# GadGadGad/Convolutional-KAN-for-Image-Classification

Measured on AMD Instinct MI355X. Metric: images/sec fwd+bwd KAN-VGG11 3x32x32 bs=256/GPU, higher is better.
Workload: dtype f32

## Files before the change

### convolutional-kan-for-image-classification_amd/_lib.py

```python
from __future__ import annotations

import ctypes as C
import os
from typing import Optional

_HERE = os.path.dirname(os.path.abspath(__file__))
LIB_PATH = os.environ.get("KANCONV_LIB") or os.path.join(_HERE, "libkanconv.so")

KAN_MAX_PLANES = 16
KAN_MAX_TABLE = 32
KAN_FP_WORDS = 192
BASIS_BSPLINE, BASIS_RBF, BASIS_CHEBY, BASIS_POLY, BASIS_FOURIER, BASIS_RELU, BASIS_GRAM = 0, 1, 2, 3, 4, 5, 6
ACT_NONE, ACT_IDENTITY, ACT_GELU, ACT_SILU, ACT_RELU, ACT_TANH, ACT_SIGMOID, ACT_GELU_TANH = -1, 0, 1, 2, 3, 4, 5, 6


class KanGeom(C.Structure):
    _fields_ = [(n, C.c_int) for n in ("B", "C", "H", "W", "O", "Ho", "Wo", "kh", "kw", "sh", "sw", "ph", "pw", "dh", "dw", "groups")] + \
               [("x_bstride", C.c_longlong), ("y_bstride", C.c_longlong)]


class KanBasis(C.Structure):
    _fields_ = [("kind", C.c_int), ("n_basis", C.c_int), ("order", C.c_int), ("act", C.c_int),
                ("p0", C.c_float), ("p1", C.c_float), ("table", C.c_float * KAN_MAX_TABLE), ("chan_table", C.c_void_p)]


class KanPlan(C.Structure):
    _fields_ = [(n, C.c_int) for n in ("P", "K", "IPC", "KC", "Kpad", "Opad", "fwd_splits", "bwd_data_splits", "bwd_weight_splits",
                                          "fwd_target", "bwd_data_target", "bwd_weight_target", "x_pm_wanted", "dz_pm_wanted", "bwd_weight_expanded", "row_blocks", "e_pm_wanted", "fwd_expanded", "fwd_halo", "bwd_weight_halo",
                                          "fwd_band", "bwd_weight_band")] + \
               [(n, C.c_longlong) for n in ("packed_weight_bytes", "bwd_data_weight_bytes", "fwd_slab_elems", "bwd_data_slab_elems",
                                            "bwd_weight_slab_elems", "e_pm_elems")]


class KanWavGeom(C.Structure):
    _fields_ = [(n, C.c_int) for n in ("B", "C", "H", "W", "O", "Ho", "Wo", "kh", "kw", "sh", "sw", "ph", "pw", "dh", "dw", "wavelet")] + \
               [("x_bstride", C.c_longlong), ("u_bstride", C.c_longlong)]


WAVELETS = {"mexican_hat": 0, "morlet": 1, "dog": 2, "meyer": 3, "shannon": 4}

_P, _I, _LL, _F, _D = C.c_void_p, C.c_int, C.c_longlong, C.c_float, C.c_double
_GP, _BP = C.POINTER(KanGeom), C.POINTER(KanBasis)
SIGNATURES = {
    "kan_version": (C.c_char_p, []),
    "kan_last_error": (C.c_char_p, []),
    "kan_plan": (_I, [_GP, _BP, C.POINTER(KanPlan)]),
    "kan_pack_weights": (_I, [_P, _P, _P, _P, _GP, _BP, _P]),
    "kan_pack_cacheable": (_I, [_GP, _BP]),
    "kan_pack_weights_cached": (_I, [_P, _P, _P, _P, _GP, _BP, _P, _I, _I, _I, _P]),
    "kan_conv_fwd": (_I, [_P, _P, _P, _P, _GP, _BP, _P, _P]),
    "kan_position_major": (_I, [_P, _P, _I, _I, _I, _LL, _P]),
    "kan_conv_bwd_data": (_I, [_P, _P, _P, _P, _P, _P, _GP, _BP, _P, _P]),
    "kan_conv_bwd_data_params": (_I, [_P, _P, _P, _P, _P, _P, _P, _GP, _BP, _P, _P]),
    "kan_conv_bwd_weight": (_I, [_P, _P, _P, _P, _GP, _BP, _P, _P, _P]),
    "kan_position_major_expanded": (_I, [_P, _P, _GP, _BP, _P]),
    "kan_conv_fwd_expanded": (_I, [_P, _P, _P, _GP, _BP, _P]),
    "kan_conv_bwd_weight_expanded": (_I, [_P, _P, _P, _GP, _BP, _P]),
    "kan_unpack_wgrad": (_I, [_P, _P, _P, _GP, _BP, _P]),
    "kan_slab_reduce": (_I, [_P, _I, _LL, _P, _I, _I, _I, _LL, _P]),
    "kan_instnorm_prelu_fwd": (_I, [_P, _I, _LL, _P, _P, _P, _P, _P, _P, _P, _I, _I, _I, _LL, _F, _I, _P]),
    "kan_instnorm_prelu_bwd": (_I, [_P, _P, _P, _P, _P, _P, _P, _P, _P, _P, _P, _I, _I, _I, _LL, _I, _P]),
    "kan_instnorm_prelu_pool_fwd": (_I, [_P, _I, _LL, _P, _P, _P, _P, _P, _P, _P, _P, _I, _I, _I, _I, _LL, _F, _I, _P]),
    "kan_instnorm_prelu_pool_bwd": (_I, [_P, _P, _P, _P, _P, _P, _P, _P, _P, _P, _P, _P, _I, _I, _I, _I, _LL, _I, _P]),
    "kan_instnorm_prelu_poolk_fwd": (_I, [_P, _I, _LL, _P, _P, _P, _P, _P, _P, _P, _P, _I, _I, _I, _I, _LL, _F, _I, _I, _I, _P]),
    "kan_instnorm_prelu_poolk_bwd": (_I, [_P, _P, _P, _P, _P, _P, _P, _P, _P, _P, _P, _P, _I, _I, _I, _I, _LL, _I, _I, _I, _P]),
    "kan_split_supported": (_I, [C.POINTER(KanGeom), C.POINTER(KanBasis)]),
    "kan_split_weight_bytes": (_LL, [C.POINTER(KanGeom), C.POINTER(KanBasis)]),
    "kan_split_pack_weights": (_I, [_P, _P, _P, C.POINTER(KanGeom), C.POINTER(KanBasis), _P]),
    "kan_conv_fwd_split": (_I, [_P, _P, _P, C.POINTER(KanGeom), C.POINTER(KanBasis), _P]),
    "kan_wav_fwd": (_I, [_P, _P, _P, _P, _P, C.POINTER(KanWavGeom), _P]),
    "kan_wav_bwd_input": (_I, [_P, _P, _P, _P, _P, _P, C.POINTER(KanWavGeom), _P]),
    "kan_wav_param_workspace": (_LL, [C.POINTER(KanWavGeom)]),
    "kan_wav_bwd_params": (_I, [_P, _P, _P, _P, _P, _P, _P, _P, _P, C.POINTER(KanWavGeom), _P]),
    "kan_adamw_step": (_I, [_P, _P, _P, _P, _LL, _D, _D, _D, _D, _D, _I, _F, _P]),
    "kan_adamw_step_segments": (_I, [_P, _P, _P, _P, _P, _P, _P, _P, _P, _I, _I, _D, _D, _D, _D, _D, _I, _F, _P]),
}

_lib: Optional[C.CDLL] = None


class KanConvError(RuntimeError):
# ... 27 lines not shown
```

### convolutional-kan-for-image-classification_amd/csrc/kan_internal.h

```cpp
#pragma once
#include <type_traits>
#include "kanconv.h"

int kan_fail_msg(const char* fmt, const char* a);
int kan_raise_lds_limit(const void* kernel, int bytes);

enum : int {
    FAST_GENERIC = 0,
    FAST_BSPLINE_SILU = 1,
    FAST_BSPLINE_GELU = 2,
    FAST_RBF8 = 3,
    FAST_CHEBY5 = 4,
    FAST_CHEBY4 = 5,
    FAST_POLY4 = 6,
    FAST_POLY3 = 7,
    FAST_RBF5 = 8,
    FAST_RELU8 = 9,
    FAST_GRAM4 = 10,
    FAST_POLY1 = 11,
    FAST_LAST = 11
};
enum : unsigned {
    ON_TAP_MAJOR = 1u << 0,
    ON_BIG_TILES = 1u << 1,
    ON_HALO_FWD = 1u << 2,
    ON_HALO_BWD_WEIGHT = 1u << 3,
    ON_BAND_FWD = 1u << 4,
    ON_BAND_BWD_WEIGHT = 1u << 5,
    ON_EXPANDED_FWD = 1u << 6,
    ON_EXPANDED = 1u << 7,
    ON_ROWBLK_BWD_DATA = 1u << 8,
};
constexpr unsigned fast_routes(int f) {
    constexpr unsigned bspline = ON_TAP_MAJOR | ON_BIG_TILES | ON_HALO_FWD | ON_HALO_BWD_WEIGHT | ON_BAND_FWD | ON_BAND_BWD_WEIGHT |
                                 ON_EXPANDED_FWD | ON_EXPANDED | ON_ROWBLK_BWD_DATA;
    switch (f) {
        case FAST_BSPLINE_SILU: case FAST_BSPLINE_GELU: return bspline;
        case FAST_RBF8: return ON_TAP_MAJOR | ON_BAND_FWD | ON_BAND_BWD_WEIGHT;
        case FAST_CHEBY5: return ON_TAP_MAJOR | ON_BIG_TILES | ON_BAND_FWD | ON_BAND_BWD_WEIGHT;
        case FAST_CHEBY4: return ON_TAP_MAJOR | ON_HALO_FWD | ON_BAND_FWD;
        case FAST_POLY4: return ON_TAP_MAJOR | ON_BIG_TILES | ON_HALO_FWD | ON_BAND_FWD;
        case FAST_POLY3: case FAST_RBF5: case FAST_POLY1: return ON_TAP_MAJOR;
        case FAST_RELU8: return ON_HALO_FWD | ON_HALO_BWD_WEIGHT | ON_EXPANDED_FWD | ON_EXPANDED;
        case FAST_GRAM4: return ON_HALO_FWD | ON_HALO_BWD_WEIGHT | ON_EXPANDED;
        default: return 0;
    }
}
constexpr bool fast_has(int f, unsigned routes) { return (fast_routes(f) & routes) == routes && f != FAST_GENERIC; }
constexpr int fast_kind(int f) {
    return (f == FAST_RBF8 || f == FAST_RBF5) ? KAN_BASIS_RBF : (f == FAST_CHEBY5 || f == FAST_CHEBY4) ? KAN_BASIS_CHEBY
         : (f == FAST_POLY4 || f == FAST_POLY3 || f == FAST_POLY1) ? KAN_BASIS_POLY : f == FAST_RELU8 ? KAN_BASIS_RELU
         : f == FAST_GRAM4 ? KAN_BASIS_GRAM : KAN_BASIS_BSPLINE;
}
constexpr int fast_kc(int f) { return fast_kind(f) == KAN_BASIS_BSPLINE || fast_kind(f) == KAN_BASIS_RBF ? 18 : 16; }

template <int V> using IC = std::integral_constant<int, V>;
template <unsigned ROUTES, int F = 1, class Fn>
bool dispatch_fast(int f, Fn&& fn) {
    if constexpr (F > FAST_LAST) {
        return false;
    } else {
        if constexpr (fast_has(F, ROUTES)) {
            if (f == F) { fn(IC<F>{}); return true; }
        }
        return dispatch_fast<ROUTES, F + 1>(f, fn);
    }
}
template <int V, int... REST, class Fn>
// ... 23 lines not shown
    int lds_bytes, wgs_per_cu;
    int fwd_splits;
    int bw_ok, bw_WR, bw_NI, bw_NT, bw_tiles_o, bw_row_tiles, bw_TPI, bw_ptiles, bw_cells, bw_slots, bw_lds_bytes, bw_splits;
    unsigned short bw_ph_rt0[KAN_BAND_MAX_PHASES + 1];
    unsigned char ph_a[KAN_BAND_MAX_PHASES], ph_b[KAN_BAND_MAX_PHASES];
    short ph_tap0[KAN_BAND_MAX_PHASES + 1];
    unsigned short tap_shift[KAN_BAND_MAX_TAPS];
    unsigned short tap_rt[KAN_BAND_MAX_TAPS];
    short tap_step[KAN_BAND_MAX_TAPS], tap_nt[KAN_BAND_MAX_TAPS];
} KanBandCfg;

void kan_band_cfg(const KanGeom* g, const KanBasis* b, int fast, KanBandCfg* cfg);
int kan_band_bwd_weight_launch(const float* dz, const float* x, const float* xn, float* dwp, const KanGeom* g, const KanBasis* b,
                               const KanBandCfg* cfg, int splits, long long slab_elems, void* stream);
int kan_band_fwd_launch(const float* x, const float* xn, const float* wp, float* z, const KanGeom* g, const KanBasis* b,
                        const KanBandCfg* cfg, int splits, long long slab_elems, void* stream);

constexpr int DW_T = 9;
constexpr int DW_MAX_TP = 96;

enum class Route { TAP_MAJOR, DW, BAND, HALO, EXPANDED };

struct FwdCfg { int TO, TP, tiles_o, tiles_p, chunks, splits, slots; };
struct BdCfg { int CH, tiles_c, tiles_p, n_ob, Opad32, chunks, splits; };
struct BwCfg { int TR, TO, tiles_r, tiles_o, chunks, splits, slots; };
struct BwHaloCfg { int R, nimg, spb, n_bands, tiles_r, tiles_o, splits, bands_per_split; };

struct ConvPlan {
    KanPlan pub;
    int fast;
    Route fwd, bwd_data, bwd_weight;
    bool pm_fwd, pm_bwd_data, pm_bwd_weight;
    bool rowblk_bwd_data;
    bool pmdma_xcd, pm_lpt, pm_xcd;
    FwdCfg fc;
    BdCfg bd;
    BwCfg bw;
    BwHaloCfg bwh;
    KanBandCfg band;
};
int plan_conv(const KanGeom* g, const KanBasis* b, ConvPlan* cp);

int live_taps_out(const KanGeom* g, int hw);
int live_taps_in(const KanGeom* g, int hw);
int live_positions_for_tap(const KanGeom* g, int tap);
int balance_tiles(const int* weight, int n, unsigned short* idx);
```

### convolutional-kan-for-image-classification_amd/csrc/kan_plan.hip

```cpp
#include <hip/hip_runtime.h>
#include <cstdio>
#include <cstdlib>
#include <cstring>
#include "kanconv.h"
#include "kan_device.h"
#include "kan_common.h"
#include "kan_internal.h"

namespace {

int fail(const char* msg) { return kan_fail_msg("%s", msg); }

int check(const KanGeom* g, const KanBasis* b) {
    if (!g || !b) return fail("null geometry/basis");
    if (g->groups < 0 || g->groups > 65535) return fail("groups out of range");
    if (g->B <= 0 || g->C <= 0 || g->O <= 0 || g->H <= 0 || g->W <= 0 || g->Ho <= 0 || g->Wo <= 0) return fail("non-positive dimension");
    if (g->kh <= 0 || g->kw <= 0 || g->sh <= 0 || g->sw <= 0 || g->dh <= 0 || g->dw <= 0 || g->ph < 0 || g->pw < 0) return fail("bad conv parameters");
    if (g->kh > 255 || g->kw > 255 || g->C > 65535) return fail("kernel size / channel count out of supported range");
    if ((g->H + 2 * g->ph - g->dh * (g->kh - 1) - 1) / g->sh + 1 != g->Ho || (g->W + 2 * g->pw - g->dw * (g->kw - 1) - 1) / g->sw + 1 != g->Wo)
        return fail("Ho/Wo inconsistent with H/W, kernel, stride, padding, dilation");
    if ((long long)g->B * g->Ho * g->Wo >= (1ll << 31) || (long long)g->B * g->H * g->W >= (1ll << 31)) return fail("pixel count exceeds int32");
    if ((long long)g->B * g->x_bstride * 4 >= (1ll << 31) || (long long)g->B * g->y_bstride * 4 >= (1ll << 31))
        return fail("activation tensors must be smaller than 2 GiB (32-bit buffer offsets)");
    if (g->x_bstride < (long long)ngroups(g) * g->C * g->H * g->W || g->y_bstride < (long long)ngroups(g) * g->O * g->Ho * g->Wo)
// ... 94 lines not shown
    if (g->kh != 3 || g->kw != 3 || g->sh != 1 || g->sw != 1 || g->dh != 1 || g->dw != 1 || g->ph != 1 || g->pw != 1) return false;
    if ((g->C & 1) || g->O % 128 != 0) return false;
    if (pm_fwd) return false;
    const int W = g->W, H = g->H;
    return (W == 32 && H % 4 == 0) || (W == 16 && H % 8 == 0) || (W == 8 && H == 8) || (W == 4 && H == 4);
}
bool band_fwd(const KanGeom* g, const KanBasis* b, int f, bool dw, bool pm_fwd, bool halo, KanBandCfg* out) {
    if (tuning_off("KAN_BAND") || !fast_has(f, ON_BAND_FWD)) return false;
    if (b->kind == KAN_BASIS_POLY && b->order == 0) return false;
    if (dw || pm_fwd || halo) return false;
    if (!(g->C <= 3 || round_up(g->O, 64) % 128 != 0 || (g->kh * g->kw >= 4 && g->C % 2 == 0 && !tuning_off("KAN_BAND_WIDE")))) return false;
    kan_band_cfg(g, b, f, out);
    return out->ok != 0;
}
FwdCfg fwd_cfg(const KanGeom* g, const KanPlan& pl, bool big, bool pm_fwd, bool halo) {
    FwdCfg c;
    c.TO = (big && !pm_fwd) ? 256 : (pl.Opad % 128 == 0) ? 128 : 64;
    c.slots = c.TO == 256 ? 512 : 1024;
    c.TP = 128;
    c.tiles_o = pl.Opad / c.TO;
    c.tiles_p = ceil_div((long long)g->B * g->Ho * g->Wo, c.TP);
    c.chunks = pl.Kpad / pl.KC;
    c.splits = pick_splits((long long)c.tiles_o * c.tiles_p * ngroups(g), c.chunks, 8, 4.0 * g->B * g->O * g->Ho * g->Wo * ngroups(g), c.slots);
    if (halo) {
        const int n_pairs = g->C / 2, pps = ceil_div(n_pairs, c.splits < n_pairs ? c.splits : n_pairs);
        c.splits = ceil_div(n_pairs, pps);
    }
    return c;
}
bool rowblk_bwd_data(const KanGeom* g, int f, bool pm_bwd_data) {
    return !tuning_off("KAN_BD_ROWBLK") && fast_has(f, ON_ROWBLK_BWD_DATA) && !pm_bwd_data && g->H == 4 && g->W == 4 && g->Ho == 4 && g->Wo == 4 &&
           g->kh == 3 && g->kw == 3 && g->sh == 1 && g->sw == 1 && g->ph == 1 && g->pw == 1 && g->dh == 1 && g->dw == 1 && g->B % 8 == 0 && g->O % 16 == 0;
}
struct LiveClass { long long tiles; int live_steps; };

int pick_target_steps(const LiveClass* cls, int ncls, int min_steps, double slab_bytes, int* max_splits, long long SLOTS = 1024) {
    int hi = 1;
    for (int i = 0; i < ncls; ++i) if (cls[i].live_steps > hi) hi = cls[i].live_steps;
    int best = hi; double best_cost = -1; int best_ms = 1;
    for (int t = min_steps < hi ? min_steps : hi; t <= hi; ++t) {
        long long wgs = 0; int ms = 1;
        for (int i = 0; i < ncls; ++i) {
            const int sp = cls[i].live_steps > 0 ? ceil_div(cls[i].live_steps, t) : 1;
            wgs += cls[i].tiles * sp;
            if (sp > ms) ms = sp;
        }
        const long long rounds = (wgs + SLOTS - 1) / SLOTS;
        const double cost = (double)(rounds * (t + 6)) + ms * slab_cost_steps(slab_bytes);
        if (best_cost < 0 || cost < best_cost) { best_cost = cost; best = t; best_ms = ms; }
    }
    *max_splits = best_ms;
    return best;
}
BdCfg bd_cfg(const KanGeom* g, const KanPlan& pl) {
    BdCfg c;
    c.CH = 64 / pl.P;
    c.tiles_c = ceil_div(g->C, 2 * c.CH);
    c.tiles_p = ceil_div((long long)g->B * g->H * g->W, 128);
    c.n_ob = ceil_div(g->O, 16);
    c.Opad32 = round_up(g->O, 32);
    c.chunks = g->kh * g->kw * c.n_ob;
    c.splits = pick_splits((long long)c.tiles_c * c.tiles_p * ngroups(g), c.chunks, 8, 4.0 * g->B * g->C * g->H * g->W * ngroups(g));
    return c;
}
bool pmdma_bwd_weight(const KanGeom* g, const KanBasis* b, int f, bool want_pm_bw) {
    if (tuning_off("KAN_PMDMA") || !fast_has(f, ON_EXPANDED)) return false;
// ... 98 lines not shown
        order[j] = v;
    }
    for (int r = 0; r < n; ++r) {
        const int depth = r / 8, k = r % 8, bin = (depth & 1) ? 7 - k : k;
        int slot = depth * 8 + bin;
        if (slot >= n) slot = r;
        idx[slot] = (unsigned short)order[r];
    }
    bool seen[PERM_MAX] = {false};
    for (int i = 0; i < n; ++i) { if (idx[i] >= n || seen[idx[i]]) return 0; seen[idx[i]] = true; }
    return n;
}

int plan_conv(const KanGeom* g, const KanBasis* b, ConvPlan* cp) {
    if (int rc = check(g, b)) return rc;
    ConvPlan& c = *cp;
    KanPlan* pl = &c.pub;
    const int T = g->kh * g->kw, G = ngroups(g), f = fast_variant(b);
    c.fast = f;
    const bool pm_shape = pmdma_fwd_shape(g, f);
    c.pm_fwd = want_pix_major(g, b, PM_FWD, pm_shape);
    c.pm_bwd_data = want_pix_major(g, b, PM_BWD_DATA, false);
    const bool want_pm_bw = want_pix_major(g, b, PM_BWD_WEIGHT, false);
    const bool dw = dw_direct(g, b);
    const bool halo = halo_fwd(g, b, f, c.pm_fwd);
    c.band.ok = c.band.bw_ok = 0;
    const bool band = band_fwd(g, b, f, dw, c.pm_fwd, halo, &c.band);
    const bool pmdma_fwd = pm_shape && c.pm_fwd;
    const bool pmdma_bw = pmdma_bwd_weight(g, b, f, want_pm_bw);
    const bool halo_bw = halo_bwd_weight(g, f, pmdma_bw);
    c.pm_bwd_weight = want_pm_bw && !halo_bw;
    const bool band_bw = band && c.band.bw_ok && !want_pm_bw && !tuning_off("KAN_BAND_BW");
    c.rowblk_bwd_data = rowblk_bwd_data(g, f, c.pm_bwd_data);
    c.pmdma_xcd = tuning_on("KAN_PMDMA_XCD");
    c.pm_lpt = !tuning_off("KAN_PM_LPT");
    c.pm_xcd = !tuning_off("KAN_PM_XCD");
    c.fwd = dw ? Route::DW : band ? Route::BAND : halo ? Route::HALO : pmdma_fwd ? Route::EXPANDED : Route::TAP_MAJOR;
    c.bwd_data = dw ? Route::DW : Route::TAP_MAJOR;
    c.bwd_weight = dw ? Route::DW : band_bw ? Route::BAND : halo_bw ? Route::HALO : pmdma_bw ? Route::EXPANDED : Route::TAP_MAJOR;
    pl->P = b->n_basis + (b->act != KAN_ACT_NONE);
    pl->K = g->C * T * pl->P;
    {
        int i18 = 18 / pl->P, i16 = 16 / pl->P;
        if (i18 > 4) i18 = 4;
        if (i16 > 4) i16 = 4;
        const bool use18 = (long long)i18 * pl->P * 16 > (long long)i16 * pl->P * 18;
        pl->KC = use18 ? 18 : 16;
        pl->IPC = use18 ? i18 : i16;
        if (pl->P >= 10 && pl->P <= 12) { pl->KC = 12; pl->IPC = 1; }
        if (halo) { pl->KC = 2 * pl->P; pl->IPC = 2; }
    }
    pl->Kpad = ceil_div(g->C * T, pl->IPC) * pl->KC;
    if (band) { pl->KC = c.band.NPLE; pl->IPC = c.band.NG; pl->Kpad = c.band.n_steps * c.band.NPLE; }
    pl->Opad = round_up(g->O, 64);
    pl->packed_weight_bytes = (long long)G * pl->Kpad * pl->Opad * 4;
    c.bd = bd_cfg(g, *pl);
    pl->bwd_data_weight_bytes = (long long)G * T * c.bd.Opad32 * c.bd.tiles_c * 128 * 4;
    pl->fwd_slab_elems = (long long)g->B * g->y_bstride;
    pl->bwd_data_slab_elems = (long long)g->B * g->x_bstride;
    pl->bwd_weight_slab_elems = (long long)G * pl->K * pl->Opad;
    const bool big = big_tiles(f, *pl);
    c.fc = fwd_cfg(g, *pl, big, c.pm_fwd, halo);
    c.bw = bw_cfg(g, *pl, big, c.pm_bwd_weight);
    if (halo_bw) c.bwh = bw_halo_cfg(g, *pl);
    pl->fwd_splits = band ? c.band.fwd_splits : c.fc.splits;
    pl->bwd_data_splits = c.bd.splits;
// ... 45 lines not shown
```

### convolutional-kan-for-image-classification_amd/csrc/kanconv.hip

```cpp
#include <hip/hip_runtime.h>
#include <cstdio>
#include <cstdlib>
#include <cstring>
#include <cmath>
#include <cstdint>
#include <mutex>
#include <type_traits>
#include <vector>
#include "kanconv.h"
#include "kan_device.h"

#include "kan_common.h"
#include "kan_internal.h"

namespace {


thread_local char g_err[512] = "";
int fail(const char* fmt, const char* a = "") {
    snprintf(g_err, sizeof(g_err), fmt, a);
    return -1;
}
}
int kan_fail_msg(const char* fmt, const char* a) { return fail(fmt, a); }
// ... 557 lines not shown
            for (int r = 0; r < 16; ++r) {
                const int o = o_tile0 + w_o * 64 + mi * 32 + mfma_row(r, lane);
                if (o < g.O) zb[(size_t)o * HoWo] = acc[mi][ni][r];
            }
        }
    }
}

template <int M>
__device__ __forceinline__ void wave_reduce_scatter(float (&v)[M], int lane, int& idx, float& tot) {
    int base = 0;
    int m = M;
#pragma unroll
    for (int off = 32; off >= 1; off >>= 1) {
        if (m > 1) {
            const int h = m / 2;
            const bool up = (lane & off) != 0;
#pragma unroll
            for (int i = 0; i < M / 2; ++i) {
                if (i < h) {
                    const float keep = up ? v[h + i] : v[i], send = up ? v[i] : v[h + i];
                    v[i] = keep + __shfl_xor(send, off, 64);
                }
            }
            base += up ? h : 0;
            m = h;
        } else {
            v[0] += __shfl_xor(v[0], off, 64);
        }
    }
    idx = base; tot = v[0];
}

template <int KIND, int FAST, int RB = 0>
__global__ __launch_bounds__(256, 4) void k_conv_bwd_data(
    const float* __restrict__ dz, const float* __restrict__ x, const float* __restrict__ xn, const float* __restrict__ wd,
    float* __restrict__ dx, float* __restrict__ dxn, DevGeom g, DevBasis bs, int CH, int n_ct, int n_ob, int Opad16,
    int n_chunks, int chunks_per_split, long long slab_elems, unsigned dz_bytes, TilePerm perm, float* __restrict__ dpar) {
    constexpr int TP = 128, KD = 16, NT = 256;
    __shared__ __attribute__((aligned(16))) float smem[2 * 2 * KD * 128];
    __shared__ float sTab[KAN_MAX_TABLE];

    const int tid = threadIdx.x, lane = tid & 63;
    const int wave = __builtin_amdgcn_readfirstlane(tid >> 6);
    const int w_r = wave >> 1, w_p = wave & 1;
    const int HoWo = g.Ho * g.Wo, HW = g.H * g.W, P = bs.P;
    const int Min = g.B * HW;
    const BlockId blk = xcd_block_order(false);
    const int grp = blk.y / n_ct;
    const int px_tile0 = (perm.n ? (int)perm.idx[blk.x] : blk.x) * TP, ct = blk.y - grp * n_ct;
    const int ncol = n_ct * 128;
    const int pxl = (wave & 1) * 64 + lane, ol0 = wave >> 1;
    const bool idle_rows = (ct * 2 + w_r) * CH >= g.C;
    {
        const size_t xo = (size_t)grp * g.C * HW;
        x += xo; xn += xo; dx += xo; if (dxn) dxn += xo;
        dz += (size_t)grp * g.O * HoWo * (g.pix_major ? g.B : 1);
        wd += (size_t)grp * (g.kh * g.kw) * Opad16 * ncol;
    }

    if (tid < KAN_MAX_TABLE) sTab[tid] = bs.tab[tid];
    const int my_px = px_tile0 + (RB ? ((pxl >> 2) & 7) * 16 + (pxl >> 5) * 4 + (pxl & 3) : pxl);
    const bool pv = my_px < Min;
    int pb, ph_, pw_;
    {
        int hw;
        if (g.pix_major) { hw = my_px / g.B; pb = my_px - hw * g.B; }
        else { pb = my_px / HW; hw = my_px - pb * HW; }
        ph_ = hw / g.W; pw_ = hw - ph_ * g.W;
    }
    const kan_rsrc dz_rs = make_rsrc(dz, dz_bytes);
    const unsigned dz_img = g.pix_major ? (unsigned)pb : (unsigned)pb * (unsigned)g.ybs;
    const unsigned zstride = g.pix_major ? (unsigned)g.B : 1u;
    const int wv = wave;

    int cur_tap = -1; unsigned base = KAN_OOB;
    const unsigned wlane = (unsigned)((lane >> 5) * ncol + (lane & 31) * 4) * 4u;
    const unsigned row_bytes = (unsigned)HoWo * zstride * 4u;
    const bool o_full = (n_ob * KD == g.O);

    auto issue = [&](int ch, int buf) {
        const int tap = ch / n_ob, o0 = (ch - tap * n_ob) * KD;
        if (tap != cur_tap) {
            cur_tap = tap;
            const int r = tap / g.kw, t = tap - r * g.kw;
            const int hn = ph_ + g.ph - r * g.dh, wn = pw_ + g.pw - t * g.dw;
            int ho = hn, wo = wn; bool ok = pv && hn >= 0 && wn >= 0;
            if (g.sh != 1 || g.sw != 1) {
                ho = hn / g.sh; wo = wn / g.sw;
                ok = ok && ho * g.sh == hn && wo * g.sw == wn;
            }
            ok = ok && ho < g.Ho && wo < g.Wo;
            base = ok ? (dz_img + (unsigned)(ho * g.Wo + wo) * zstride) * 4u : KAN_OOB;
        }
        float* dW = smem + buf * (2 * KD * 128);
// ... 65 lines not shown
#pragma unroll
        for (int b = 0; b < 2; ++b)
#pragma unroll
            for (int r = 0; r < 16; ++r) acc[a][b][r] = 0.f;

    int ch0 = blk.z * chunks_per_split;
    int ch1 = min(n_chunks, ch0 + chunks_per_split);
    unsigned tapmask = 0xffffffffu;
    if (g.pix_major) {
        tapmask = 0;
        const int T = g.kh * g.kw;
        const int hwA = px_tile0 / g.B, hwB = min(px_tile0 + TP - 1, Min - 1) / g.B;
        for (int hw = hwA; hw <= hwB; ++hw)
            for (int tap = 0; tap < T; ++tap) tapmask |= (tap_alive_in(g, hw, tap) ? 1u : 0u) << tap;
        auto seg = [&](int tap) { return tap * n_ob; };
        const int L = live_step_count(tapmask, T, n_chunks, seg);
        const int S = min((int)gridDim.z, max(1, (L + chunks_per_split - 1) / chunks_per_split));
        if (blk.z >= S) { ch0 = ch1 = n_chunks; }
        else {
            ch0 = blk.z == 0 ? 0 : live_step_pos(tapmask, T, n_chunks, (int)((long long)L * blk.z / S), seg);
            ch1 = blk.z == S - 1 ? n_chunks : live_step_pos(tapmask, T, n_chunks, (int)((long long)L * (blk.z + 1) / S), seg);
        }
    }
    auto next_live = [&](int ch) -> int {
        if (!g.pix_major) return ch;
        while (ch < ch1) {
            const int tap = ch / n_ob;
            if ((tapmask >> tap) & 1u) return ch;
            ch = (tap + 1) * n_ob;
        }
        return ch1;
    };
    int ch = next_live(ch0);
    if (ch < ch1) { if (RB) issue_rb(ch, 0); else issue(ch, 0); }
    const int ar = w_r * 64 + (lane & 31), bp = w_p * 64 + (lane & 31), kh2 = lane >> 5;
    for (int cur = 0; ch < ch1; cur ^= 1) {
        asm volatile("s_waitcnt vmcnt(0)" ::: "memory");
        __syncthreads();
        const bool mixed_now = pend_mixed;
        ch = next_live(ch + 1);
        if (ch < ch1) { if (RB) issue_rb(ch, cur ^ 1); else issue(ch, cur ^ 1); }
        const float* cW = smem + cur * (2 * KD * 128);
        const float* cG = cW + KD * 128;
        const unsigned aw = lds_addr(cW + kh2 * 128 + ar), ag = lds_addr(cG + kh2 * TP + bp);
        if (RB) {
            const bool l0b = !(mixed_now && w_p == 0), l1a = !(mixed_now && w_p == 1);
            if (!idle_rows) KAN_MFMA_STEP_LIVE(KD / 2, aw, 128, ag, TP, true, l0b, l1a, true);
        } else if (!idle_rows) KAN_MFMA_STEP(KD / 2, aw, 128, ag, TP);
    }

    const bool same_in = (x == xn);
    const bool split_out = (dxn != nullptr);
    float* dxs = dx + (size_t)blk.z * slab_elems;
    float* dxns = split_out ? dxn + (size_t)blk.z * slab_elems : nullptr;
    if (FAST == 3 || FAST == 8) {
        constexpr int FP = FAST == 3 ? 9 : 6, FCH = 64 / FP, NIT = (FCH + 1) / 2;
        const float inv_d = 1.0f / bs.p0;
#pragma unroll 1
        for (int half = 0; half < 2; ++half) {
            float xv[NIT], nv[NIT]; unsigned ok = 0;
#pragma unroll
            for (int it = 0; it < NIT; ++it) {
                const int cl = ol0 + 2 * it, c = (ct * 2 + half) * FCH + cl;
                const bool v = cl < FCH && c < g.C && pv;
                const size_t idx = (size_t)pb * g.xbs + (size_t)c * HW + (size_t)(ph_ * g.W + pw_);
                xv[it] = v ? x[idx] : 0.f;
                nv[it] = v ? xn[idx] : 0.f;
                ok |= (v ? 1u : 0u) << it;
// ... 1676 lines not shown
    if (pl.KC != pl.IPC * pl.P || (pl.fwd_band && pack_needs_clear(g, pl))) {
        if (hipMemsetAsync(wp, 0, (size_t)pl.packed_weight_bytes, st) != hipSuccess) return fail("memset failed");
    } else if (!pl.fwd_band && NI % pl.IPC != 0) {
        if (G > 1) {
            if (hipMemsetAsync(wp, 0, (size_t)pl.packed_weight_bytes, st) != hipSuccess) return fail("memset failed");
        } else {
            size_t off = (size_t)(pl.Kpad - pl.KC) * pl.Opad;
            if (hipMemsetAsync(wp + off, 0, (size_t)pl.KC * pl.Opad * 4, st) != hipSuccess) return fail("memset failed");
        }
    }
    const int nb_base = hb ? ceil_div(g->C * T, 32) : 0;
    const int tiles_x = nb_base + ceil_div(g->C * b->n_basis * T, 32), tiles_y = pl.Opad / 32;
    const long long n_tiles = (long long)tiles_x * tiles_y;
    const long long cap = fp ? 1024 : 4096;
    dim3 grid((unsigned)(n_tiles < cap ? n_tiles : cap), 1, G);
    hipLaunchKernelGGL(k_pack, grid, dim3(256), 0, st, w_base, w_basis, wp, q, nb_base, wp_gs, tiles_x, tiles_y, fp, fp_cur);
    if (wd && cp.bwd_data == Route::DW) {
        if (hipMemcpyAsync(wd, wp, (size_t)pl.packed_weight_bytes, hipMemcpyDeviceToDevice, st) != hipSuccess) return fail("memcpy failed");
    } else if (wd) {
        const BdCfg& c = cp.bd;
        const int bx = c.tiles_c * 4, by = c.Opad32 / 32 * G;
        const long long nt = (long long)bx * by;
        const long long capd = fp ? 128 : 1024;
        dim3 gd((unsigned)(nt < capd ? nt : capd), 1, T);
        hipLaunchKernelGGL(k_pack_bwd_data, gd, dim3(256), 0, st, (const float*)wp, wd, q, c.CH, c.tiles_c, c.Opad32, wp_gs, bx, by, fp, fp_cur);
    }
    return launch_ok("pack");
}

int kan_pack_weights(const float* w_base, const float* w_basis, float* wp, float* wd, const KanGeom* g, const KanBasis* b, void* stream) {
    return pack_weights_impl(w_base, w_basis, wp, wd, g, b, nullptr, 0, stream);
}

int kan_pack_cacheable(const KanGeom* g, const KanBasis* b) {
    ConvPlan cp;
    if (plan_conv(g, b, &cp)) return 0;
    if ((long long)g->O * g->C * (b->n_basis + 1) * g->kh * g->kw >= (1ll << 31)) return 0;
    return (!pack_needs_clear(g, cp.pub) && cp.fwd != Route::DW && ngroups(g) == 1) ? 1 : 0;
}

int kan_pack_weights_cached(const float* w_base, const float* w_basis, float* wp, float* wd, const KanGeom* g, const KanBasis* b,
                            unsigned long long* ring, int cur, int force, int sample_stride, void* stream) {
    static_assert(KAN_FP_WORDS == 3 * FP_LANES, "ring size");
    if (!ring || cur < 0 || cur > 2 || sample_stride < 1) return fail("bad fingerprint ring arguments");
    if (!kan_pack_cacheable(g, b)) return fail("cached packing is not offered for this geometry (kan_pack_cacheable)");
    const int hb = b->act != KAN_ACT_NONE;
    if ((hb && !w_base) || !w_basis) return fail("null weight pointer");
    if (((size_t)w_basis & 15) || (hb && ((size_t)w_base & 15))) return fail("cached packing needs 16-byte aligned weight tensors");
    const int T = g->kh * g->kw;
    const long long na = hb ? (long long)g->O * g->C * T : 0, nbs = (long long)g->O * g->C * b->n_basis * T;
    const long long groups4 = ((na + 3) / 4 + (nbs + 3) / 4 + sample_stride - 1) / sample_stride;
    long long blocks = (groups4 + 256 * 8 - 1) / (256 * 8); if (blocks > 4096) blocks = 4096; if (blocks < 1) blocks = 1;
    hipLaunchKernelGGL(k_fingerprint, dim3((unsigned)blocks), dim3(256), 0, (hipStream_t)stream, hb ? w_base : w_basis, (unsigned)na, w_basis,
                       (unsigned)nbs, (unsigned)sample_stride, ring, cur);
    if (int rc = launch_ok("fingerprint")) return rc;
    return pack_weights_impl(w_base, w_basis, wp, wd, g, b, force ? nullptr : ring, cur, stream);
}

int kan_unpack_wgrad(const float* dwp, float* dw_base, float* dw_basis, const KanGeom* g, const KanBasis* b, void* stream) {
    ConvPlan cp;
    if (int rc = plan_conv(g, b, &cp)) return rc;
    const KanPlan& pl = cp.pub;
    const int hb = b->act != KAN_ACT_NONE;
    if ((hb && !dw_base) || !dw_basis || !dwp) return fail("null weight-gradient pointer");
    hipStream_t st = (hipStream_t)stream;
    const int T = g->kh * g->kw, G = ngroups(g);
// ... 121 lines not shown
    ConvPlan cp;
    if (int rc = plan_conv(g, b, &cp)) return rc;
    const KanPlan& pl = cp.pub;
    if (dpar && cp.bwd_data == Route::DW) return fail("kan_conv_bwd_data_params: depthwise layers take the weight-gradient route");
    if (!dz || !x || !xn || !wd || !dx) return fail("null tensor pointer");
    if ((b->kind == KAN_BASIS_RELU || b->kind == KAN_BASIS_GRAM) && !b->chan_table) return fail("ReLU / Gram bases need their device parameter table (chan_table)");
    if (!dxn && x != xn) return fail("dxn is required when xn != x");
    hipStream_t st = (hipStream_t)stream;
    if (cp.bwd_data == Route::DW) {
        DevGeom dgd = dev_geom(g); DevBasis dbd = dev_basis(b);
        dim3 grid(ceil_div((long long)g->B * g->H * g->W, 256), ngroups(g));
        dispatch_kind(b->kind, [&](auto kind) {
            hipLaunchKernelGGL((k_dw_bwd_data<decltype(kind)::value>), grid, dim3(256), 0, st, dz, x, xn, wd, dx, dxn, dgd, dbd, pl.Opad, pl.IPC, pl.KC, pl.Kpad);
        });
        return launch_ok("dw_bwd_data");
    }
    const BdCfg& c = cp.bd;
    DevGeom dg = dev_geom(g);
    dg.pix_major = (dz_pm && cp.pm_bwd_data) ? 1 : 0;
    if (dg.pix_major) dz = dz_pm;
    DevBasis db = dev_basis(b);
    if ((long long)c.tiles_c * ngroups(g) > 65535) return fail("groups * channel tiles exceed the grid limit");
    dim3 grid(c.tiles_p, c.tiles_c * ngroups(g), pl.bwd_data_splits);
    const int cps = dg.pix_major ? pl.bwd_data_target : ceil_div(c.chunks, pl.bwd_data_splits);
    TilePerm perm; perm.n = 0;
    if (dg.pix_major) perm = tile_perm(c.tiles_p, [&](int t) {
        const int hw = (int)(((long long)t * 128) / g->B);
        return ceil_div(live_taps_in(g, hw < g->H * g->W ? hw : 0) * c.n_ob, cps > 0 ? cps : 1);
    });
    const int fv = cp.fast;
    const int fast = (fv == FAST_RBF8 || fv == FAST_RBF5) ? ((x != xn && dxn) ? fv : 0) : ((x == xn && !dxn) ? fv : 0);
    const bool rb = !dg.pix_major && cp.rowblk_bwd_data;
    const unsigned dz_bytes = (unsigned)((long long)g->B * g->y_bstride * 4);
    auto launch = [&](auto kind, auto fast, auto rbv) {
        hipLaunchKernelGGL((k_conv_bwd_data<decltype(kind)::value, decltype(fast)::value, decltype(rbv)::value>), grid, dim3(256), 0, st, dz, x, xn, wd,
                           dx, dxn, dg, db, c.CH, c.tiles_c, c.n_ob, c.Opad32, c.chunks, cps, pl.bwd_data_slab_elems, dz_bytes, perm, dpar);
    };
    const bool launched = dispatch_fast<ON_TAP_MAJOR>(fast, [&](auto fv) {
        constexpr int F = decltype(fv)::value;
        if constexpr (fast_has(F, ON_ROWBLK_BWD_DATA)) {
            if (rb) return launch(IC<fast_kind(F)>{}, fv, IC<1>{});
        }
        launch(IC<fast_kind(F)>{}, fv, IC<0>{});
    });
    if (!launched) dispatch_kind(b->kind, [&](auto kind) { launch(kind, IC<FAST_GENERIC>{}, IC<0>{}); });
    return launch_ok("conv_bwd_data");
}

int kan_conv_bwd_weight(const float* dz, const float* x, const float* xn, float* dwp, const KanGeom* g, const KanBasis* b,
                        const float* x_pm, const float* dz_pm, void* stream) {
    ConvPlan cp;
    if (int rc = plan_conv(g, b, &cp)) return rc;
    const KanPlan& pl = cp.pub;
    if (!dz || !x || !xn || !dwp) return fail("null tensor pointer");
    if ((b->kind == KAN_BASIS_RELU || b->kind == KAN_BASIS_GRAM) && !b->chan_table) return fail("ReLU / Gram bases need their device parameter table (chan_table)");
    hipStream_t st = (hipStream_t)stream;
    if (cp.bwd_weight == Route::DW) {
        DevGeom dgd = dev_geom(g); DevBasis dbd = dev_basis(b);
        dim3 grid(pl.bwd_weight_splits, ngroups(g));
        dispatch_kind(b->kind, [&](auto kind) {
            hipLaunchKernelGGL((k_dw_bwd_weight<decltype(kind)::value>), grid, dim3(256), 0, st, dz, x, xn, dwp, dgd, dbd, pl.K, pl.Opad, pl.bwd_weight_slab_elems);
        });
        return launch_ok("dw_bwd_weight");
    }
    if (cp.bwd_weight == Route::BAND) {
        if (x != xn && b->kind != KAN_BASIS_RBF && b->kind != KAN_BASIS_POLY) return fail("this basis / activation pair runs on single-input kernels: pass xn == x");
        return kan_band_bwd_weight_launch(dz, x, xn, dwp, g, b, &cp.band, pl.bwd_weight_splits, pl.bwd_weight_slab_elems, stream);
    }
    const unsigned x_bytes = (unsigned)((long long)g->B * g->x_bstride * 4), dz_bytes = (unsigned)((long long)g->B * g->y_bstride * 4);
    if (cp.bwd_weight == Route::HALO) {
        if (x != xn) return fail("internal: the channel-major weight-gradient layout needs x == xn");
        const BwHaloCfg& hc = cp.bwh;
        const DevGeom dgh = dev_geom(g); const DevBasis dbh = dev_basis(b);
        if ((long long)hc.tiles_o * ngroups(g) > 65535) return fail("groups * output tiles exceed the grid limit");
        dim3 grid(hc.tiles_r, hc.tiles_o * ngroups(g), hc.splits);
        dispatch_fast<ON_HALO_BWD_WEIGHT>(cp.fast, [&](auto fv) {
            auto launch = [&](auto w, auto r, auto nimg) {
                hipLaunchKernelGGL((k_conv_bwd_weight_halo<decltype(fv)::value, decltype(w)::value, decltype(r)::value, decltype(nimg)::value>), grid,
// ... 286 lines not shown
```

### include/kanconv.h

```cpp
#ifndef KANCONV_H
#define KANCONV_H

#ifdef __cplusplus
extern "C" {
#endif

#define KAN_MAX_PLANES 16
#define KAN_MAX_TABLE  32
#define KAN_FP_WORDS   192

enum { KAN_BASIS_BSPLINE = 0, KAN_BASIS_RBF = 1, KAN_BASIS_CHEBY = 2, KAN_BASIS_POLY = 3, KAN_BASIS_FOURIER = 4, KAN_BASIS_RELU = 5, KAN_BASIS_GRAM = 6 };
enum { KAN_ACT_NONE = -1, KAN_ACT_IDENTITY = 0, KAN_ACT_GELU = 1, KAN_ACT_SILU = 2, KAN_ACT_RELU = 3,
       KAN_ACT_TANH = 4, KAN_ACT_SIGMOID = 5, KAN_ACT_GELU_TANH = 6 };

typedef struct KanGeom {
    int B, C, H, W;
    int O, Ho, Wo;
    int kh, kw, sh, sw, ph, pw, dh, dw;
    int groups;
    long long x_bstride;
    long long y_bstride;
} KanGeom;

typedef struct KanBasis {
// ... 5 lines not shown

typedef struct KanPlan {
    int P;
    int K;
    int IPC, KC;
    int Kpad, Opad;
    int fwd_splits;
    int bwd_data_splits;
    int bwd_weight_splits;
    int fwd_target, bwd_data_target, bwd_weight_target;
    int x_pm_wanted, dz_pm_wanted;
    int bwd_weight_expanded;
    int row_blocks;
    int e_pm_wanted, fwd_expanded;
    int fwd_halo, bwd_weight_halo;
    int fwd_band, bwd_weight_band;
    long long packed_weight_bytes;
    long long bwd_data_weight_bytes;
    long long fwd_slab_elems;
    long long bwd_data_slab_elems;
    long long bwd_weight_slab_elems;
    long long e_pm_elems;
} KanPlan;

const char* kan_version(void);
const char* kan_last_error(void);

int kan_plan(const KanGeom* geom, const KanBasis* basis, KanPlan* plan);

int kan_pack_weights(const float* w_base, const float* w_basis, float* wp, float* wd,
                     const KanGeom* geom, const KanBasis* basis, void* stream);

int kan_pack_cacheable(const KanGeom* geom, const KanBasis* basis);
int kan_pack_weights_cached(const float* w_base, const float* w_basis, float* wp, float* wd,
                            const KanGeom* geom, const KanBasis* basis, unsigned long long* ring, int cur, int force,
                            int sample_stride, void* stream);

int kan_conv_fwd(const float* x, const float* xn, const float* wp, float* z,
                 const KanGeom* geom, const KanBasis* basis, const float* x_pm, void* stream);

int kan_position_major(const float* src, float* dst, int B, int Cn, int HW, long long bstride, void* stream);

int kan_conv_bwd_data(const float* dz, const float* x, const float* xn, const float* wd,
                      float* dx, float* dxn,
                      const KanGeom* geom, const KanBasis* basis, const float* dz_pm, void* stream);

int kan_conv_bwd_data_params(const float* dz, const float* x, const float* xn, const float* wd, float* dx, float* dxn, float* dparams,
                             const KanGeom* geom, const KanBasis* basis, const float* dz_pm, void* stream);

int kan_conv_bwd_weight(const float* dz, const float* x, const float* xn, float* dwp,
                        const KanGeom* geom, const KanBasis* basis, const float* x_pm, const float* dz_pm, void* stream);

int kan_position_major_expanded(const float* x, float* e_pm, const KanGeom* geom, const KanBasis* basis, void* stream);
int kan_conv_fwd_expanded(const float* e_pm, const float* wp, float* z, const KanGeom* geom, const KanBasis* basis, void* stream);
int kan_conv_bwd_weight_expanded(const float* dz_pm, const float* e_pm, float* dwp,
                                 const KanGeom* geom, const KanBasis* basis, void* stream);

int kan_unpack_wgrad(const float* dwp, float* dw_base, float* dw_basis,
                     const KanGeom* geom, const KanBasis* basis, void* stream);

int kan_slab_reduce(const float* slabs, int n_slabs, long long slab_elems, float* out,
                    int B, int Cn, int HW, long long bstride, void* stream);

int kan_instnorm_prelu_fwd(const float* z, int n_slabs, long long slab_elems, float* z_out,
                           const float* gamma, const float* beta, const float* prelu_a,
                           float* y, float* mean, float* rstd,
// ... 55 lines not shown
```

Measured before the change: 17270.

## Add halo-staged LDS path for 4x4 row-blocked backward-data conv

Adds a HALO template variant of the backward-data kernel. For 4x4 3x3 layers on the row-block route, it stages a padded halo tile of dz into LDS once per output-channel block and reads all nine taps from shifted LDS offsets, instead of re-gathering dz for each tap. Tap slots are paired and the nine-slot loop is unrolled with compile-time offsets, and MFMAs on known-dead rows are skipped. This raises LDS use and code complexity, and it only applies to the small 4x4 layers of the network.

```diff
diff --git a/convolutional-kan-for-image-classification_amd/_lib.py b/convolutional-kan-for-image-classification_amd/_lib.py
--- a/convolutional-kan-for-image-classification_amd/_lib.py
+++ b/convolutional-kan-for-image-classification_amd/_lib.py
@@ -47,6 +47,7 @@
     "kan_plan": (_I, [_GP, _BP, C.POINTER(KanPlan)]),
     "kan_pack_weights": (_I, [_P, _P, _P, _P, _GP, _BP, _P]),
     "kan_pack_cacheable": (_I, [_GP, _BP]),
+    "kan_bwd_data_halo": (_I, [_GP, _BP]),
     "kan_pack_weights_cached": (_I, [_P, _P, _P, _P, _GP, _BP, _P, _I, _I, _I, _P]),
     "kan_conv_fwd": (_I, [_P, _P, _P, _P, _GP, _BP, _P, _P]),
     "kan_position_major": (_I, [_P, _P, _I, _I, _I, _LL, _P]),
diff --git a/convolutional-kan-for-image-classification_amd/csrc/kan_internal.h b/convolutional-kan-for-image-classification_amd/csrc/kan_internal.h
--- a/convolutional-kan-for-image-classification_amd/csrc/kan_internal.h
+++ b/convolutional-kan-for-image-classification_amd/csrc/kan_internal.h
@@ -30,10 +30,11 @@
     ON_EXPANDED_FWD = 1u << 6,
     ON_EXPANDED = 1u << 7,
     ON_ROWBLK_BWD_DATA = 1u << 8,
+    ON_HALO_BWD_DATA = 1u << 9,
 };
 constexpr unsigned fast_routes(int f) {
     constexpr unsigned bspline = ON_TAP_MAJOR | ON_BIG_TILES | ON_HALO_FWD | ON_HALO_BWD_WEIGHT | ON_BAND_FWD | ON_BAND_BWD_WEIGHT |
-                                 ON_EXPANDED_FWD | ON_EXPANDED | ON_ROWBLK_BWD_DATA;
+                                 ON_EXPANDED_FWD | ON_EXPANDED | ON_ROWBLK_BWD_DATA | ON_HALO_BWD_DATA;
     switch (f) {
         case FAST_BSPLINE_SILU: case FAST_BSPLINE_GELU: return bspline;
         case FAST_RBF8: return ON_TAP_MAJOR | ON_BAND_FWD | ON_BAND_BWD_WEIGHT;
@@ -123,6 +124,7 @@
     Route fwd, bwd_data, bwd_weight;
     bool pm_fwd, pm_bwd_data, pm_bwd_weight;
     bool rowblk_bwd_data;
+    bool halo_bwd_data;
     bool pmdma_xcd, pm_lpt, pm_xcd;
     FwdCfg fc;
     BdCfg bd;
diff --git a/convolutional-kan-for-image-classification_amd/csrc/kan_plan.hip b/convolutional-kan-for-image-classification_amd/csrc/kan_plan.hip
--- a/convolutional-kan-for-image-classification_amd/csrc/kan_plan.hip
+++ b/convolutional-kan-for-image-classification_amd/csrc/kan_plan.hip
@@ -150,6 +150,9 @@
     return !tuning_off("KAN_BD_ROWBLK") && fast_has(f, ON_ROWBLK_BWD_DATA) && !pm_bwd_data && g->H == 4 && g->W == 4 && g->Ho == 4 && g->Wo == 4 &&
            g->kh == 3 && g->kw == 3 && g->sh == 1 && g->sw == 1 && g->ph == 1 && g->pw == 1 && g->dh == 1 && g->dw == 1 && g->B % 8 == 0 && g->O % 16 == 0;
 }
+bool halo_bwd_data(const KanGeom* g, int f, bool pm_bwd_data) {
+    return !tuning_off("KAN_BD_HALO") && fast_has(f, ON_HALO_BWD_DATA) && rowblk_bwd_data(g, f, pm_bwd_data);
+}
 struct LiveClass { long long tiles; int live_steps; };
 
 int pick_target_steps(const LiveClass* cls, int ncls, int min_steps, double slab_bytes, int* max_splits, long long SLOTS = 1024) {
@@ -314,6 +317,7 @@
     c.pm_bwd_weight = want_pm_bw && !halo_bw;
     const bool band_bw = band && c.band.bw_ok && !want_pm_bw && !tuning_off("KAN_BAND_BW");
     c.rowblk_bwd_data = rowblk_bwd_data(g, f, c.pm_bwd_data);
+    c.halo_bwd_data = !dw && halo_bwd_data(g, f, c.pm_bwd_data);
     c.pmdma_xcd = tuning_on("KAN_PMDMA_XCD");
     c.pm_lpt = !tuning_off("KAN_PM_LPT");
     c.pm_xcd = !tuning_off("KAN_PM_XCD");
diff --git a/convolutional-kan-for-image-classification_amd/csrc/kanconv.hip b/convolutional-kan-for-image-classification_amd/csrc/kanconv.hip
--- a/convolutional-kan-for-image-classification_amd/csrc/kanconv.hip
+++ b/convolutional-kan-for-image-classification_amd/csrc/kanconv.hip
@@ -613,13 +613,59 @@
     idx = base; tot = v[0];
 }
 
-template <int KIND, int FAST, int RB = 0>
+template <int W> struct BdHalo {
+    static constexpr int R = W == 32 ? 4 : W == 16 ? 8 : W == 8 ? 8 : 4, NIMG = 128 / (R * W);
+    static constexpr int HWc = W == 16 ? 24 : W + 2, HIMG = W == 8 ? 112 : (R + 2) * HWc, CELLS = NIMG * HIMG;
+    static constexpr int NI = (CELLS + 63) / 64, PITCH = NI * 64;
+    static constexpr int FLOATS = 2 * 16 * 128 + 16 * PITCH > 64 * 128 ? 2 * 16 * 128 + 16 * PITCH : 64 * 128;
+};
+template <> struct BdHalo<0> { static constexpr int FLOATS = 2 * 2 * 16 * 128; };
+__host__ __device__ constexpr int bdh_tap_lo(int slot) { return slot == 4 ? 5 : slot < 4 ? slot : slot - 5; }
+__host__ __device__ constexpr int bdh_tap_hi(int slot) { return slot == 4 ? 5 : (slot % 5) < 3 ? (slot % 5) + 6 : 4; }
+__host__ __device__ constexpr int bdh_half_lo(int slot) { return slot > 4 ? 1 : 0; }
+__host__ __device__ constexpr int bdh_half_hi(int slot) { return slot >= 4 ? 1 : 0; }
+template <int W, int RB>
+__device__ __forceinline__ void bdh_pixel(int n, int& img, int& row, int& col) {
+    if (RB) { row = n >> 5; img = (n >> 2) & 7; col = n & 3; }
+    else if (W == 16) { img = 0; row = (n >> 6) * 4 + ((n >> 3) & 3); col = ((n >> 5) & 1) * 8 + (n & 7); }
+    else if (W == 8) { img = (n >> 4) & 1; row = (n >> 5) + 4 * ((n >> 3) & 1); col = n & 7; }
+    else { constexpr int PI = BdHalo<W>::R * W; img = n / PI; row = (n - img * PI) / W; col = n % W; }
+}
+template <int W, int RB> constexpr int bdh_d32() { return RB ? BdHalo<W>::HWc : W == 16 ? 8 : W == 4 ? 2 * BdHalo<W>::HIMG : BdHalo<W>::HWc; }
+#define KAN_MFMA_STEP_HALO(addrA, addrBl, addrBh, LO, HI, PB, D32, l0a, l0b, l1a, l1b)                                                \
+    do {                                                                                                                           \
+        float fa_[2][2], fb_[2][2];                                                                                                \
+        LDS_READ4(fa_[0][0], fa_[0][1], fb_[0][0], fb_[0][1], addrA, addrBl, 0, 32 * 4, (LO), (LO) + (D32));                       \
+        _Pragma("unroll") for (int kk = 0; kk < 8; ++kk) {                                                                          \
+            const int c_ = kk & 1, n_ = c_ ^ 1;                                                                                    \
+            if (kk + 1 < 4) {                                                                                                      \
+                LDS_READ4(fa_[n_][0], fa_[n_][1], fb_[n_][0], fb_[n_][1], addrA, addrBl, (2 * (kk + 1)) * 128 * 4,                 \
+                          (2 * (kk + 1)) * 128 * 4 + 128, (LO) + 2 * ((kk + 1) & 3) * (PB), (LO) + 2 * ((kk + 1) & 3) * (PB) + (D32)); \
+                LDS_WAIT4(fa_[c_][0], fa_[c_][1], fb_[c_][0], fb_[c_][1], 4);                                                      \
+            } else if (kk + 1 < 8) {                                                                                               \
+                LDS_READ4(fa_[n_][0], fa_[n_][1], fb_[n_][0], fb_[n_][1], addrA, addrBh, (2 * (kk + 1)) * 128 * 4,                 \
+                          (2 * (kk + 1)) * 128 * 4 + 128, (HI) + 2 * ((kk + 1) & 3) * (PB), (HI) + 2 * ((kk + 1) & 3) * (PB) + (D32)); \
+                LDS_WAIT4(fa_[c_][0], fa_[c_][1], fb_[c_][0], fb_[c_][1], 4);                                                      \
+            } else {                                                                                                               \
+                LDS_WAIT4(fa_[c_][0], fa_[c_][1], fb_[c_][0], fb_[c_][1], 0);                                                      \
+            }                                                                                                                      \
+            if (kk < 4 ? (l0a) : (l0b)) {                                                                                          \
+                acc[0][0] = MFMA32(fa_[c_][0], fb_[c_][0], acc[0][0]);                                                             \
+                acc[1][0] = MFMA32(fa_[c_][1], fb_[c_][0], acc[1][0]);                                                             \
+            }                                                                                                                      \
+            if (kk < 4 ? (l1a) : (l1b)) {                                                                                          \
+                acc[0][1] = MFMA32(fa_[c_][0], fb_[c_][1], acc[0][1]);                                                             \
+                acc[1][1] = MFMA32(fa_[c_][1], fb_[c_][1], acc[1][1]);                                                             \
+            }                                                                                                                      \
+        }                                                                                                                          \
+    } while (0)
+template <int KIND, int FAST, int RB = 0, int HALO = 0>
 __global__ __launch_bounds__(256, 4) void k_conv_bwd_data(
     const float* __restrict__ dz, const float* __restrict__ x, const float* __restrict__ xn, const float* __restrict__ wd,
     float* __restrict__ dx, float* __restrict__ dxn, DevGeom g, DevBasis bs, int CH, int n_ct, int n_ob, int Opad16,
     int n_chunks, int chunks_per_split, long long slab_elems, unsigned dz_bytes, TilePerm perm, float* __restrict__ dpar) {
     constexpr int TP = 128, KD = 16, NT = 256;
-    __shared__ __attribute__((aligned(16))) float smem[2 * 2 * KD * 128];
+    __shared__ __attribute__((aligned(16))) float smem[BdHalo<HALO>::FLOATS];
     __shared__ float sTab[KAN_MAX_TABLE];
 
     const int tid = threadIdx.x, lane = tid & 63;
@@ -641,7 +687,12 @@
     }
 
     if (tid < KAN_MAX_TABLE) sTab[tid] = bs.tab[tid];
-    const int my_px = px_tile0 + (RB ? ((pxl >> 2) & 7) * 16 + (pxl >> 5) * 4 + (pxl & 3) : pxl);
+    int my_px = px_tile0 + (RB ? ((pxl >> 2) & 7) * 16 + (pxl >> 5) * 4 + (pxl & 3) : pxl);
+    if constexpr (HALO > 0) {
+        int im, rw, cl;
+        bdh_pixel<HALO, RB>(pxl, im, rw, cl);
+        my_px = px_tile0 + im * (BdHalo<HALO>::R * HALO) + rw * HALO + cl;
+    }
     const bool pv = my_px < Min;
     int pb, ph_, pw_;
     {
@@ -773,8 +824,100 @@
         return ch1;
     };
     int ch = next_live(ch0);
-    if (ch < ch1) { if (RB) issue_rb(ch, 0); else issue(ch, 0); }
     const int ar = w_r * 64 + (lane & 31), bp = w_p * 64 + (lane & 31), kh2 = lane >> 5;
+    if constexpr (HALO > 0) {
+        using HT = BdHalo<HALO>;
+        constexpr int PITCH = HT::PITCH, HWc = HT::HWc;
+        float* const sH = smem + 2 * KD * 128;
+        const int b0 = px_tile0 / HW, h0 = (px_tile0 - b0 * HW) / HALO;
+        unsigned hoff[HT::NI];
+#pragma unroll
+        for (int c = 0; c < HT::NI; ++c) {
+            const int cell = c * 64 + lane, img = cell / HT::HIMG, rem = cell - img * HT::HIMG, hr = rem / HWc, hc = rem - hr * HWc;
+            const int bb = b0 + img, hh_ = h0 + hr - 1, ww = hc - 1;
+            const bool okc = cell < HT::CELLS && bb < g.B && hh_ >= 0 && hh_ < g.H && ww >= 0 && ww < HALO;
+            hoff[c] = okc ? ((unsigned)bb * (unsigned)g.ybs + (unsigned)(hh_ * HALO + ww)) * 4u : KAN_OOB;
+        }
+        auto stage = [&](int hf, int ob) {
+#pragma unroll
+            for (int n = 0; n < 2; ++n) {
+                const int ol = hf * 8 + wv + 4 * n;
+                const unsigned so = (unsigned)(ob * KD + ol) * row_bytes;
+#pragma unroll
+                for (int c = 0; c < HT::NI; ++c)
+                    __builtin_amdgcn_raw_ptr_buffer_load_lds(dz_rs, (__attribute__((address_space(3))) void*)(sH + ol * PITCH + c * 64), 4,
+                                                             (int)hoff[c], (int)so, 0, 0);
+            }
+        };
+        auto issue_w = [&](int ob, int slot, int buf) {
+            const int rlo = bdh_tap_lo(slot) * Opad16 + ob * KD + bdh_half_lo(slot) * 8 + wv * 2;
+            const int rhi = bdh_tap_hi(slot) * Opad16 + ob * KD + bdh_half_hi(slot) * 8 + wv * 2;
+            float* dW = smem + buf * (KD * 128);
+            glds16((const float*)((const char*)(wd + (size_t)rlo * ncol + ct * 128) + wlane), dW + wv * 256);
+            glds16((const float*)((const char*)(wd + (size_t)rhi * ncol + ct * 128) + wlane), dW + (4 + wv) * 256);
+        };
+        int cell0;
+        {
+            int im, rw, cl;
+            bdh_pixel<HALO, RB>(w_p * 64 + (lane & 31), im, rw, cl);
+            cell0 = im * HT::HIMG + rw * HWc + cl;
+        }
+        constexpr int D32 = bdh_d32<HALO, RB>() * 4;
+        const unsigned ag = lds_addr(sH + kh2 * PITCH + cell0);
+        const unsigned aw0 = lds_addr(smem + kh2 * 128 + ar);
+        if (ch0 < ch1) {
+            const int ob0 = ch0 / 9, sl0 = ch0 - ob0 * 9;
+            stage(1, ob0);
+            if (sl0 <= 4) stage(0, ob0);
+            else if ((ob0 + 1) * 9 < ch1) stage(0, ob0 + 1);
+            issue_w(ob0, sl0, 0);
+        }
+        unsigned cur = 0;
+        auto pre = [&](int s, int ob, int sl) __attribute__((always_inline)) {
+            asm volatile("s_waitcnt vmcnt(0)" ::: "memory");
+            __syncthreads();
+            if (s + 1 < ch1) issue_w(sl == 8 ? ob + 1 : ob, sl == 8 ? 0 : sl + 1, (int)(cur ^ 1u));
+            if (sl == 0 && s != ch0) stage(1, ob);
+            if (sl == 5 && s != ch0 && (ob + 1) * 9 < ch1) stage(0, ob + 1);
+        };
+        const bool dead0b = RB && w_p == 0, dead1a = RB && w_p == 1;
+        int s = ch0;
+        auto part = [&](int end) __attribute__((always_inline)) {
+#pragma unroll 1
+            for (; s < end; ++s) {
+                const int ob = s / 9, sl = s - ob * 9;
+                pre(s, ob, sl);
+                const int tl = bdh_tap_lo(sl), th = bdh_tap_hi(sl);
+                const unsigned agl = ag + (unsigned)((bdh_half_lo(sl) * 8 * PITCH + (2 - tl / 3) * HWc + (2 - tl % 3)) * 4);
+                const unsigned agh = ag + (unsigned)((bdh_half_hi(sl) * 8 * PITCH + (2 - th / 3) * HWc + (2 - th % 3)) * 4);
+                const bool mixed = tl / 3 == 0 && th / 3 == 2;
+                const unsigned aw = aw0 + cur * (KD * 128 * 4);
+                if (!idle_rows) KAN_MFMA_STEP_HALO(aw, agl, agh, 0, 0, PITCH * 4, D32, true, !(mixed && dead0b), !(mixed && dead1a), true);
+                cur ^= 1u;
+            }
+        };
+        part(min(ch1, (ch0 + 8) / 9 * 9));
+#pragma unroll 1
+        for (; s + 9 <= ch1; s += 9) {
+            const int ob = s / 9;
+            auto slot = [&](auto SLc) __attribute__((always_inline)) {
+                constexpr int SL = decltype(SLc)::value;
+                pre(s + SL, ob, SL);
+                constexpr int tl = bdh_tap_lo(SL), th = bdh_tap_hi(SL);
+                constexpr int LO = (bdh_half_lo(SL) * 8 * PITCH + (2 - tl / 3) * HWc + (2 - tl % 3)) * 4;
+                constexpr int HI = (bdh_half_hi(SL) * 8 * PITCH + (2 - th / 3) * HWc + (2 - th % 3)) * 4;
+                constexpr bool mixed = tl / 3 == 0 && th / 3 == 2;
+                const unsigned aw = aw0 + cur * (KD * 128 * 4);
+                if (!idle_rows) KAN_MFMA_STEP_HALO(aw, ag, ag, LO, HI, PITCH * 4, D32, true, !(mixed && dead0b), !(mixed && dead1a), true);
+                cur ^= 1u;
+            };
+            slot(IC<0>{}); slot(IC<1>{}); slot(IC<2>{}); slot(IC<3>{}); slot(IC<4>{}); slot(IC<5>{}); slot(IC<6>{}); slot(IC<7>{}); slot(IC<8>{});
+        }
+        part(ch1);
+        asm volatile("s_waitcnt vmcnt(0)" ::: "memory");
+        ch = ch1;
+    }
+    if (HALO == 0 && ch < ch1) { if (RB) issue_rb(ch, 0); else issue(ch, 0); }
     for (int cur = 0; ch < ch1; cur ^= 1) {
         asm volatile("s_waitcnt vmcnt(0)" ::: "memory");
         __syncthreads();
@@ -2517,6 +2660,12 @@
     return pack_weights_impl(w_base, w_basis, wp, wd, g, b, nullptr, 0, stream);
 }
 
+int kan_bwd_data_halo(const KanGeom* g, const KanBasis* b) {
+    ConvPlan cp;
+    if (int rc = plan_conv(g, b, &cp)) return rc;
+    return cp.halo_bwd_data ? 1 : 0;
+}
+
 int kan_pack_cacheable(const KanGeom* g, const KanBasis* b) {
     ConvPlan cp;
     if (plan_conv(g, b, &cp)) return 0;
@@ -2704,18 +2853,22 @@
     const int fast = (fv == FAST_RBF8 || fv == FAST_RBF5) ? ((x != xn && dxn) ? fv : 0) : ((x == xn && !dxn) ? fv : 0);
     const bool rb = !dg.pix_major && cp.rowblk_bwd_data;
     const unsigned dz_bytes = (unsigned)((long long)g->B * g->y_bstride * 4);
-    auto launch = [&](auto kind, auto fast, auto rbv) {
-        hipLaunchKernelGGL((k_conv_bwd_data<decltype(kind)::value, decltype(fast)::value, decltype(rbv)::value>), grid, dim3(256), 0, st, dz, x, xn, wd,
-                           dx, dxn, dg, db, c.CH, c.tiles_c, c.n_ob, c.Opad32, c.chunks, cps, pl.bwd_data_slab_elems, dz_bytes, perm, dpar);
+    auto launch = [&](auto kind, auto fast, auto rbv, auto halo_w) {
+        hipLaunchKernelGGL((k_conv_bwd_data<decltype(kind)::value, decltype(fast)::value, decltype(rbv)::value, decltype(halo_w)::value>), grid, dim3(256),
+                           0, st, dz, x, xn, wd, dx, dxn, dg, db, c.CH, c.tiles_c, c.n_ob, c.Opad32, c.chunks, cps, pl.bwd_data_slab_elems, dz_bytes,
+                           perm, dpar);
     };
     const bool launched = dispatch_fast<ON_TAP_MAJOR>(fast, [&](auto fv) {
         constexpr int F = decltype(fv)::value;
+        if constexpr (fast_has(F, ON_HALO_BWD_DATA | ON_ROWBLK_BWD_DATA)) {
+            if (rb && cp.halo_bwd_data) return launch(IC<fast_kind(F)>{}, fv, IC<1>{}, IC<4>{});
+        }
         if constexpr (fast_has(F, ON_ROWBLK_BWD_DATA)) {
-            if (rb) return launch(IC<fast_kind(F)>{}, fv, IC<1>{});
-        }
-        launch(IC<fast_kind(F)>{}, fv, IC<0>{});
+            if (rb) return launch(IC<fast_kind(F)>{}, fv, IC<1>{}, IC<0>{});
+        }
+        launch(IC<fast_kind(F)>{}, fv, IC<0>{}, IC<0>{});
     });
-    if (!launched) dispatch_kind(b->kind, [&](auto kind) { launch(kind, IC<FAST_GENERIC>{}, IC<0>{}); });
+    if (!launched) dispatch_kind(b->kind, [&](auto kind) { launch(kind, IC<FAST_GENERIC>{}, IC<0>{}, IC<0>{}); });
     return launch_ok("conv_bwd_data");
 }
 
diff --git a/include/kanconv.h b/include/kanconv.h
--- a/include/kanconv.h
+++ b/include/kanconv.h
@@ -61,6 +61,7 @@
                      const KanGeom* geom, const KanBasis* basis, void* stream);
 
 int kan_pack_cacheable(const KanGeom* geom, const KanBasis* basis);
+int kan_bwd_data_halo(const KanGeom* geom, const KanBasis* basis);
 int kan_pack_weights_cached(const float* w_base, const float* w_basis, float* wp, float* wd,
                             const KanGeom* geom, const KanBasis* basis, unsigned long long* ring, int cur, int force,
                             int sample_stride, void* stream);
```

New measurement: 17330, median of 6. No clear change (+0.3%).
